# stresearch/xfr

Hardware: AMD Instinct MI355X
Metric: triplet-contrastive-EBP saliency maps/sec, ResNet-101 224x224 (higher is better)
Workload: dtype f32

## Files before the change

### xfr_amd/csrc/conv_gemm.hip

```cpp
#include <algorithm>
#include <atomic>
#include <mutex>
#include <unordered_map>
#include <vector>
#include "common.h"
#include <cstdio>
#include <cstdlib>

#include "conv_gemm_dev.h"
#include "conv_gemm_host.h"

std::atomic<long> g_conv_chain_launches[2];

namespace {

#ifndef XFR_MFM_WAVES
#define XFR_MFM_WAVES 6
#endif
#ifndef XFR_DUAL_WAVES
#define XFR_DUAL_WAVES 4
#endif
template <int TCO, int TM, int BK, int NST, int MODE, bool RELU, int CHAIN>
__global__ __launch_bounds__(NT, CHAIN == 0 ? 1 : (CHAIN == 1 ? 7 : (CHAIN == 4 ? XFR_DUAL_WAVES : XFR_MFM_WAVES))) void conv_gemm_kernel(const ConvParams p, const int n_co_tiles, const int n_m_tiles)
{
// ... 491 lines not shown
            if (kk + 2 < BK) {
#pragma unroll
                for (int i = 0; i < 2; ++i) { a_nxt[i] = As[(kk + 2 + lhi) * TCO + l31 + i * 32]; b_nxt[i] = Bs[(kk + 2 + lhi) * TM + l31 + i * 32]; }
            } else {
                wait_vmcnt<(NST - 2) * L>();
                const float* An = ring + st_next * STAGE;
#pragma unroll
                for (int i = 0; i < 2; ++i) { a_nxt[i] = An[lhi * TCO + l31 + i * 32]; b_nxt[i] = An[A_FLOATS + lhi * TM + l31 + i * 32]; }
            }
            if (RELU) { b_cur[0] = fmaxf(b_cur[0], 0.f); b_cur[1] = fmaxf(b_cur[1], 0.f); }
#pragma unroll
            for (int i = 0; i < 2; ++i)
#pragma unroll
                for (int j = 0; j < 2; ++j) acc[i][j] = __builtin_amdgcn_mfma_f32_32x32x2f32(a_cur[i], b_cur[j], acc[i][j], 0, 0, 0);
            if constexpr (DUAL) {
                const float ap0 = fmaxf(a_cur[0], 0.f), ap1 = fmaxf(a_cur[1], 0.f);
#pragma unroll
                for (int j = 0; j < 2; ++j) {
                    accp[0][j] = __builtin_amdgcn_mfma_f32_32x32x2f32(ap0, b_cur[j], accp[0][j], 0, 0, 0);
                    accp[1][j] = __builtin_amdgcn_mfma_f32_32x32x2f32(ap1, b_cur[j], accp[1][j], 0, 0, 0);
                }
            }
            if (kk + 2 < BK) issue(kt + NST - 1, st_fill, kk / 2);
            __builtin_amdgcn_sched_group_barrier(0x100, 2, 0);
            __builtin_amdgcn_sched_group_barrier(0x008, 1, 0);
            __builtin_amdgcn_sched_group_barrier(0x020, (L + NP - 1) / NP, 0);
            __builtin_amdgcn_sched_group_barrier(0x008, DUAL ? 7 : 3, 0);
#pragma unroll
            for (int i = 0; i < 2; ++i) { a_cur[i] = a_nxt[i]; b_cur[i] = b_nxt[i]; }
        }
        st = st_next;
        asm volatile("" ::: "memory");
    }
    wait_vmcnt<0>();
    stamp(p, wave, lane, 2);

    asm volatile("s_waitcnt lgkmcnt(0)" ::: "memory");
    v16f accq[1][1];
    if (wave == 0) ks_exchange<0, WAVE_LDS>(smem, acc, lane, accq[0][0]);
    else if (wave == 1) ks_exchange<1, WAVE_LDS>(smem, acc, lane, accq[0][0]);
    else if (wave == 2) ks_exchange<2, WAVE_LDS>(smem, acc, lane, accq[0][0]);
    else ks_exchange<3, WAVE_LDS>(smem, acc, lane, accq[0][0]);
    v16f accpq;
    if constexpr (DUAL) {
        __syncthreads();
        if (wave == 0) ks_exchange<0, WAVE_LDS>(smem, accp, lane, accpq);
        else if (wave == 1) ks_exchange<1, WAVE_LDS>(smem, accp, lane, accpq);
        else if (wave == 2) ks_exchange<2, WAVE_LDS>(smem, accp, lane, accpq);
        else ks_exchange<3, WAVE_LDS>(smem, accp, lane, accpq);
    }
    stamp(p, wave, lane, 3);
    block_epilogue<CHAIN, true>(p, accq, smem, tid, lane, wave, co0, m0, half, tail_t, part, nparts, osel, bsel, DUAL ? &accpq : nullptr);
    stamp(p, wave, lane, 4);
}


int num_cus()
{
    static const int n = [] {
        int dev = 0, cu = 0;
        if (hipGetDevice(&dev) != hipSuccess || hipDeviceGetAttribute(&cu, hipDeviceAttributeMultiprocessorCount, dev) != hipSuccess || cu <= 0)
            cu = 256;
        return cu;
    }();
    return n;
}

int pick_tail_split(const ConvParams& p, int tiles, int nk, size_t tile_bytes)
{
    constexpr int qmax = 7;
    if (!p.tail_ws || !p.tail_cnt || p.tail_force == 1) return 1;
    const int C = num_cus();
    const int q = tiles / C, r = tiles % C;
    if (r == 0 || r > XFR_TAIL_MAX_TILES) return 1;
    const long max_blocks = (long)(p.tail_ws_bytes / tile_bytes);
    if (p.tail_force >= 2) {
        const int S = std::min(p.tail_force, nk);
        return ((long)r * S <= max_blocks) ? S : 1;
    }
    if (q == 0 && p.K >= 8192 && p.tail_force == 0) {
        const long S = std::min<long>(std::min<long>(64, p.K / 256), std::min<long>(max_blocks / r, std::max<long>(8, C / r)));
        return (int)std::min<long>(S, nk);
    }
    if (q >= qmax || p.K < 1024) return 1;
    const double ramp = 192.0 / (double)p.K;
    const double whole = 1.0 + ramp;
    double best = whole;
    int bestS = 1;
    const int Smax = std::min(std::min(8, p.K / 256), nk);
    for (int S = 2; S <= Smax; ++S) {
        if ((long)r * S > max_blocks) break;
        const double per_cu = (double)(((long)r * S + C - 1) / C);
        const double cost = per_cu * (1.0 / S + ramp) + 0.01 * S;
        if (cost < best) { best = cost; bestS = S; }
    }
    if (whole - best < 0.04 * (q + 1) * whole) bestS = 1;
    return bestS;
}

void warn_interpreted(const ConvParams& q)
{
    static std::atomic<int> said{0};
    const int ohw = q.OH * q.OW;
    const bool vec_ok = (q.M & 3) == 0 && ((q.chain_B * ohw) & 3) == 0 && ((q.out_nb * ohw) & 3) == 0;
    if (q.chain_interpret || !vec_ok || getenv("XFR_QUIET") || said.exchange(1)) return;
    uint16_t codes[XFR_MAX_EW_STEPS];
    const int n = ew_chain_codes(q.chain, codes);
    fprintf(stderr, "xfr_amd: a GEMM launch (Cout %d, K %d, M %d) runs its %d-step fused chain through the INTERPRETED epilogue: no compiled signature [", q.CoutTot, q.K, q.M, q.chain.n);
    for (int i = 0; i < n; ++i) fprintf(stderr, "%s%04x", i ? " " : "", codes[i]);
    fprintf(stderr, "]%s.  Regenerate the table (python tools/gen_chain_sigs.py && make -C xfr_amd/csrc) if this network is a supported backbone; "
                    "xfr_chain_epilogue_stats counts such launches.  (said once; XFR_QUIET=1 silences it)\n",
            n < 0 ? " (the chain carries a trace / prior / capture: interpreted by design)" : (q.accumulate ? " for an accumulating launch" : ""));
}

int plan_chain(ConvParams& q)
{
    EwChain wide = q.chain;
    EwLoads wide_ld;
    ew_plan_loads(wide, q.out0, wide_ld, EW_FWD_SLOTS_WIDE);
    ew_plan_loads(q.chain, q.out0, q.chain_ld);
    const int ohw = q.OH * q.OW;
    const bool vec_ok = (q.M & 3) == 0 && ((q.chain_B * ohw) & 3) == 0 && ((q.out_nb * ohw) & 3) == 0;
    q.chain_sig = (q.accumulate || !vec_ok || q.chain_interpret) ? -1 : conv_gemm_chain_sig(wide);
    if (q.chain_sig >= 0) { q.chain = wide; q.chain_ld = wide_ld; }
    if (q.nhalves == 2 && q.chain_sig < 0) return 1;
    if ((q.dualacc != 0) != (q.chain_sig >= 0 && chain_sig_is_dual(q.chain_sig))) return 3;
    for (int i = 0; i < q.chain.n && q.chain_sig < 0; ++i)
        if (q.chain.s[i].type == EW_MAXPAIR || q.chain.s[i].type == EW_MAXHALF_OUT) return 2;
    return 0;
}

template <int TCO, int TM, int BK, int NST, int MODE>
bool launch_one(const ConvParams& p, hipStream_t s)
{
    const int n_co = ((p.CoutTot + TCO - 1) / TCO) * p.nhalves;
    const int n_m = (p.M + TM - 1) / TM;
    const size_t lds = std::max((size_t)NST * BK * (TCO + TM) * sizeof(float) + (MODE == MODE_GEN ? 512 * sizeof(int2) : 0), (size_t)4 * 32 * 36 * sizeof(float));
    ConvParams q = p;
    int grid = n_co * n_m;
    q.tail_q = 0;
    q.tail_s = 1;
    {
        const int S = pick_tail_split(p, n_co * n_m, (p.K + BK - 1) / BK, (size_t)TCO * TM * sizeof(float) * (p.dualacc ? 2 : 1));
        if (S > 1) {
            const int r = (n_co * n_m) % num_cus();
            q.tail_q = n_co * n_m - r;
            q.tail_s = S;
            grid = q.tail_q + r * S;
        }
    }
    if (p.dualacc && (q.chain.n == 0 || p.nhalves != 1 || p.relu_in)) return false;
    if constexpr ((TCO == 64 && TM == 64) || (TCO == 32 && TM == 128)) {
        if (q.chain.n > 0) {
            if (plan_chain(q)) return false;
            g_conv_chain_launches[q.chain_sig >= 0 ? 0 : 1]++;
            if (q.chain_sig < 0) warn_interpreted(q);
            if constexpr (TCO == 64 && MODE != MODE_TAP4 && MODE != MODE_GEN) {
                if (q.dualacc) {
                    hipLaunchKernelGGL((conv_gemm_kernel<TCO, TM, BK, NST, MODE, false, 4>), dim3(grid), dim3(NT), lds, s, q, n_co, n_m);
                    return true;
                }
            }
            if (q.dualacc) return false;
            if (q.chain_sig >= 0 && chain_sig_is_mfm(q.chain_sig))
                hipLaunchKernelGGL((conv_gemm_kernel<TCO, TM, BK, NST, MODE, false, 3>), dim3(grid), dim3(NT), lds, s, q, n_co, n_m);
            else if (q.chain_sig >= 0)
                hipLaunchKernelGGL((conv_gemm_kernel<TCO, TM, BK, NST, MODE, false, 1>), dim3(grid), dim3(NT), lds, s, q, n_co, n_m);
            else
                hipLaunchKernelGGL((conv_gemm_kernel<TCO, TM, BK, NST, MODE, false, 2>), dim3(grid), dim3(NT), lds, s, q, n_co, n_m);
            return true;
        }
    }
    if (p.relu_in)
        hipLaunchKernelGGL((conv_gemm_kernel<TCO, TM, BK, NST, MODE, true, 0>), dim3(grid), dim3(NT), lds, s, q, n_co, n_m);
    else
        hipLaunchKernelGGL((conv_gemm_kernel<TCO, TM, BK, NST, MODE, false, 0>), dim3(grid), dim3(NT), lds, s, q, n_co, n_m);
    return true;
}

template <int BK, int NST, int MODE>
bool launch_one_ks(const ConvParams& p, hipStream_t s)
{
    constexpr int TCO = 64, TM = 64;
    const int n_co = ((p.CoutTot + TCO - 1) / TCO) * p.nhalves;
    const int n_m = (p.M + TM - 1) / TM;
    constexpr int RING = NST * BK * (TCO + TM);
    const size_t lds = (size_t)4 * (RING > 2048 ? RING : 2048) * sizeof(float);
    ConvParams q = p;
    int grid = n_co * n_m;
    q.tail_q = 0;
    q.tail_s = 1;
    {
        const int S = pick_tail_split(p, n_co * n_m, (p.K + BK - 1) / BK, (size_t)TCO * TM * sizeof(float) * (p.dualacc ? 2 : 1));
        if (S > 1) {
            const int r = (n_co * n_m) % num_cus();
            q.tail_q = n_co * n_m - r;
            q.tail_s = S;
            grid = q.tail_q + r * S;
        }
    }
    if (p.dualacc && (q.chain.n == 0 || p.nhalves != 1 || p.relu_in)) return false;
    if (q.chain.n > 0) {
        if (plan_chain(q)) return false;
        g_conv_chain_launches[q.chain_sig >= 0 ? 0 : 1]++;
        if (q.chain_sig < 0) warn_interpreted(q);
        if (q.dualacc) {
            hipLaunchKernelGGL((conv_gemm_ks_kernel<BK, NST, MODE, false, 4>), dim3(grid), dim3(NT), lds, s, q, n_co, n_m);
            return true;
        }
        if (q.chain_sig >= 0 && chain_sig_is_mfm(q.chain_sig))
            hipLaunchKernelGGL((conv_gemm_ks_kernel<BK, NST, MODE, false, 3>), dim3(grid), dim3(NT), lds, s, q, n_co, n_m);
        else if (q.chain_sig >= 0)
            hipLaunchKernelGGL((conv_gemm_ks_kernel<BK, NST, MODE, false, 1>), dim3(grid), dim3(NT), lds, s, q, n_co, n_m);
        else
            hipLaunchKernelGGL((conv_gemm_ks_kernel<BK, NST, MODE, false, 2>), dim3(grid), dim3(NT), lds, s, q, n_co, n_m);
        return true;
    }
    if (p.relu_in)
        hipLaunchKernelGGL((conv_gemm_ks_kernel<BK, NST, MODE, true, 0>), dim3(grid), dim3(NT), lds, s, q, n_co, n_m);
    else
        hipLaunchKernelGGL((conv_gemm_ks_kernel<BK, NST, MODE, false, 0>), dim3(grid), dim3(NT), lds, s, q, n_co, n_m);
    return true;
}

template <int BK>
bool ks_ok(const ConvParams& p)
{
    if ((p.Cin % BK) != 0) return false;
    if (p.kh == 1 && p.kw == 1) return p.pad == 0 && p.stride <= 2;
    if (p.out_stride != 1) return false;
    return p.stride == 1 && p.tap_major == 1 && p.kh * p.kw <= 64;
}

template <int BK, int NST>
bool launch_cfg_ks(const ConvParams& p, hipStream_t s)
{
    const bool vec = (p.kh == 1 && p.kw == 1 && p.stride == 1 && p.pad == 0 && (p.M % 4) == 0 && p.OH == p.H && p.OW == p.W);
    if (vec) return launch_one_ks<BK, NST, MODE_VEC>(p, s);
    return launch_one_ks<BK, NST, MODE_TAP>(p, s);
}


template <int TCO, int TM, int BK, int NST>
bool launch_cfg(const ConvParams& p_in, hipStream_t s)
{
    ConvParams p = p_in;
    if (p.dualacc && p.kh == 1 && p.kw == 1 && p.tap_major == 0 && (p.Cin % 16) == 0) p.tap_major = 1;
    const bool vec = (p.kh == 1 && p.kw == 1 && p.stride == 1 && p.pad == 0 && (p.M % 4) == 0 && p.OH == p.H && p.OW == p.W);
    if (vec) return launch_one<TCO, TM, BK, NST, MODE_VEC>(p, s);
    if (p.tap_major == 2) return launch_one<64, 64, 16, 4, MODE_TAP4>(p, s);
    if (p.tap_major && (p.Cin % BK) == 0) return launch_one<TCO, TM, BK, NST, MODE_TAP>(p, s);
    if (p.tap_major) return launch_one<TCO, TM, 16, 4, MODE_TAP>(p, s);
    return launch_one<TCO, TM, 16, 4, MODE_GEN>(p, s);
}

}

int conv_gemm_num_cus() { return num_cus(); }
int conv_gemm_plan_chain(ConvParams& q) { return plan_chain(q); }
void conv_gemm_warn_interpreted(const ConvParams& q) { warn_interpreted(q); }

int conv_gemm_chain_sig(const EwChain& ch)
{
    uint16_t codes[XFR_MAX_EW_STEPS];
    const int n = ew_chain_codes(ch, codes);
    if (n <= 0) return -1;
    for (int sgi = 0; sgi < kNumChainSigs; ++sgi) {
        bool same = true;
        for (int i = 0; i < XFR_MAX_EW_STEPS && same; ++i) same = kChainSigs[sgi][i] == (i < n ? codes[i] : 0);
        if (same) return sgi;
    }
    return -1;
}
int conv_gemm_num_chain_sigs() { return kNumChainSigs; }

int conv_gemm_cannot_launch(const ConvParams& p)
{
    if (p.chain.n <= 0) return 0;
    ConvParams q = p;
    return plan_chain(q);
}
const char* conv_gemm_refusal(int why)
{
    switch (why) {
        case 0: return "the convolution launch was refused without a reason";
        case 1: return "a dual (W / relu(W)) convolution launch carries a fused chain without a compiled epilogue";
        case 3: return "lean probe-forward steps and the dual-accumulator launch (ConvParams::dualacc) only exist together, behind a compiled epilogue";
        case 2: return "a fused chain with a MaxFeatureMap step (pair maximum / fan-out VJP) has no compiled epilogue and the interpreter does not run those steps";
        default: return "unknown convolution launch refusal";
    }
}

void conv_gemm_chain_launch_counts(long* compiled, long* interpreted)
{
    if (compiled) *compiled = g_conv_chain_launches[0].load();
    if (interpreted) *interpreted = g_conv_chain_launches[1].load();
}

static int pick_cfg_impl(const ConvParams& p_in, bool allow_split);
int conv_gemm_pick_cfg(const ConvParams& p_in) { return pick_cfg_impl(p_in, true); }
static int pick_cfg_impl(const ConvParams& p_in, bool allow_split)
{
    ConvParams p = p_in;
    if (p.dualacc) { p.nhalves = 2; p.dualacc = 0; const int c = pick_cfg_impl(p, false); return c == 12 ? 4 : c; }
    if (allow_split && p.split_ok && conv_gemm_split_wanted(p)) return 9;
    {
        const int rem = p.CoutTot % 64;
#ifndef XFR_NO_ROW_TILE
        if (rem > 0 && rem <= 32 && p.tap_major != 2 && p.out_stride == 1 && p.CoutTot > 32 && p.M > 64) return 12;
#endif
    }
    if (ks_ok<8>(p)) {
        if (p.kh == 1 && (p.stride == 2 || p.out_stride == 2 || p.as_strided)) return 7;
        if ((p.kh > 1 && p.K >= 2048) || (p.kh == 1 && (p.K == 512 || p.K >= 2048))) return 7;
    }
    const long tiles = (long)((p.CoutTot + 63) / 64) * p.nhalves * ((p.M + 63) / 64);
    if (p.K >= 1024 && tiles <= 512 && (p.tap_major ? (p.Cin % 32 == 0) : true)) return 5;
    return 4;
}

static std::mutex g_tune_mu;
static thread_local int g_last_cfg = 0;
static std::atomic<int> g_tuning{0};
static unsigned long long* g_stamps = nullptr;
static int g_stamps_cap = 0;
static int g_stamp_regions = 0, g_stamp_seq = 0;
namespace {
struct LogRec { void* stream; int cout, nhalves, K, M, kh, chain, cfg; };
unsigned long long* g_log = nullptr;
int g_log_cap = 0;
std::vector<LogRec> g_log_recs;
bool g_log_on() { return g_log != nullptr; }
}
void conv_gemm_set_stamps(unsigned long long* dev_ptr, int capacity_workgroups)
{
    std::lock_guard<std::mutex> lk(g_tune_mu);
    g_stamps = dev_ptr;
    g_stamps_cap = dev_ptr ? (capacity_workgroups < 0 ? -capacity_workgroups : capacity_workgroups) : 0;
    g_stamp_regions = (dev_ptr && capacity_workgroups < 0) ? (-capacity_workgroups) / 256 : 0;
    g_stamp_seq = 0;
    g_tuning.store((g_stamps || g_log_on()) ? 1 : 0);
}

void conv_gemm_set_log(unsigned long long* log_dev, int capacity)
{
    std::lock_guard<std::mutex> lk(g_tune_mu);
    g_log = log_dev;
    g_log_cap = log_dev ? capacity : 0;
    g_log_recs.clear();
    g_tuning.store((g_stamps || g_log) ? 1 : 0);
}
int conv_gemm_dump_log(const char* path)
{
    std::lock_guard<std::mutex> lk(g_tune_mu);
    if (!g_log) return 0;
    const size_t n = g_log_recs.size();
    std::vector<unsigned long long> h(8 * n + 8);
    if (n && hipMemcpy(h.data(), g_log, 8 * n * sizeof(unsigned long long), hipMemcpyDeviceToHost) != hipSuccess) return -1;
    FILE* f = fopen(path, "w");
    if (!f) return -1;
    fprintf(f, "seq,stream,Cout,nhalves,K,M,kh,chain,cfg,start_10ns,end_10ns\n");
    for (size_t i = 0; i < n; ++i) {
        const LogRec& r = g_log_recs[i];
        fprintf(f, "%zu,%p,%d,%d,%d,%d,%d,%d,%d,%llu,%llu\n", i, r.stream, r.cout, r.nhalves, r.K, r.M, r.kh, r.chain, r.cfg, h[8 * i], *std::max_element(h.begin() + 8 * i + 1, h.begin() + 8 * i + 8));
    }
    fclose(f);
    return (int)n;
}

bool launch_conv_gemm(const ConvParams& p_in, hipStream_t s)
{
    ConvParams p = p_in;
    p.stamps = nullptr;
    p.stamps_cap = 0;
    p.stamp_regions = 0;
    p.stamp_seq = 0;
    p.span = nullptr;
    size_t log_idx = (size_t)-1;
    if (g_tuning.load(std::memory_order_relaxed)) {
        std::lock_guard<std::mutex> lk(g_tune_mu);
        p.stamps = g_stamps;
        p.stamps_cap = g_stamps_cap;
        p.stamp_regions = g_stamp_regions;
        p.stamp_seq = g_stamps ? g_stamp_seq++ : 0;
        if (g_log && (int)g_log_recs.size() < g_log_cap) {
            p.span = g_log + 8 * g_log_recs.size();
            log_idx = g_log_recs.size();
            g_log_recs.push_back(LogRec{(void*)s, p.CoutTot, p.dualacc ? 2 : p.nhalves, p.K, p.M, p.kh, p.chain.n, -1});
        }
    }
    int cfg = p.force_cfg > 0 ? p.force_cfg : conv_gemm_pick_cfg(p);
    {
        struct Remap { int v[32]; };
        static const Remap remap = [] {
            Remap r;
            for (int i = 0; i < 32; ++i) r.v[i] = i;
            if (const char* e = getenv("XFR_CFG_REMAP")) {
                int a = 0, b = 0, n = 0;
                while (sscanf(e, "%d:%d%n", &a, &b, &n) == 2) {
                    if (a >= 0 && a < 32 && b >= 0 && b < 32) r.v[a] = b;
                    e += n;
                    if (*e == ',') ++e;
                }
            }
            return r;
        }();
        if (p.force_cfg <= 0 && cfg >= 0 && cfg < 32) cfg = remap.v[cfg];
    }
    auto ran = [&](int eff, bool ok) {
        g_last_cfg = eff;
        if (log_idx != (size_t)-1) {
            std::lock_guard<std::mutex> lk(g_tune_mu);
            if (log_idx < g_log_recs.size()) g_log_recs[log_idx].cfg = eff;
        }
        return ok;
    };
    if (cfg == 9) {
        if (conv_gemm_launch_split(p, s)) return ran(9, true);
        cfg = pick_cfg_impl(p, false);
    }
    if (cfg == 6 && ks_ok<8>(p)) return ran(6, launch_cfg_ks<8, 3>(p, s));
    if (cfg == 7 && ks_ok<4>(p)) return ran(7, launch_cfg_ks<4, 4>(p, s));
    if (cfg == 5) return ran(5, launch_cfg<64, 64, 32, 3>(p, s));
    if (cfg == 12) return ran(12, launch_cfg<32, 128, 16, 3>(p, s));
    return ran(4, launch_cfg<64, 64, 16, 3>(p, s));
}

int conv_gemm_last_cfg() { return g_last_cfg; }
```

### xfr_amd/csrc/conv_gemm_split.hip

```cpp
#include <algorithm>
#include <atomic>
#include <mutex>
#include <unordered_map>
#include <cstdio>
#include <cstdlib>
#include <type_traits>
#include "conv_gemm_dev.h"
#include "conv_gemm_host.h"

namespace {

typedef __bf16 v8bf __attribute__((ext_vector_type(8)));
typedef unsigned v4u __attribute__((ext_vector_type(4)));
constexpr int SP_T = 128, SP_BK = 16;
constexpr int SP_A_BYTES = 3 * 2 * SP_T * 16, SP_B_BYTES = 3 * 2 * SP_T * 16;
constexpr size_t SP_LDS = 3 * (size_t)(SP_A_BYTES + SP_B_BYTES);

typedef float v2f_t __attribute__((ext_vector_type(2)));
typedef __bf16 v2bf_t __attribute__((ext_vector_type(2)));
__device__ __forceinline__ unsigned cvt_pk_bf16(float lo, float hi)
{
    const v2f_t t = {lo, hi};
    return __builtin_bit_cast(unsigned, __builtin_convertvector(t, v2bf_t));
}
__device__ __forceinline__ void split_pair(float a, float b, unsigned& p0, unsigned& p1, unsigned& p2)
{
    p0 = cvt_pk_bf16(a, b);
    const float ra = a - __uint_as_float(p0 << 16), rb = b - __uint_as_float(p0 & 0xffff0000u);
    p1 = cvt_pk_bf16(ra, rb);
    const float sa = ra - __uint_as_float(p1 << 16), sb = rb - __uint_as_float(p1 & 0xffff0000u);
    p2 = cvt_pk_bf16(sa, sb);
}

constexpr int SPP_MAX_HALO = 64, SPP_MAX_TAPS = 25;

__host__ __device__ inline int spp_halo(const ConvParams& p) { return p.pad * p.W + p.pad; }
__host__ __device__ inline int spp_patch_len(const ConvParams& p) { return SP_T + 2 * spp_halo(p); }
inline size_t spp_lds_bytes(const ConvParams& p) { return (size_t)3 * SP_A_BYTES + (size_t)2 * 6 * (spp_patch_len(p) + 1) * 16; }

constexpr int NT8 = 512;

template <int N>
__device__ __forceinline__ void sp8_wait_barrier()
{
    asm volatile("s_waitcnt vmcnt(%0) lgkmcnt(0)\n\ts_barrier" ::"n"(N) : "memory");
}

template <bool RELU, int CHAIN, bool PATCH>
__global__ __launch_bounds__(NT8, 2) void conv_gemm_split_kernel(const ConvParams p, const uint16_t* __restrict__ ws0, const uint16_t* __restrict__ ws1,
                                                                  const int n_co_tiles, const int n_m_tiles)
{
    extern __shared__ __attribute__((aligned(16))) float smem[];
    unsigned char* lds = reinterpret_cast<unsigned char*>(smem);
    constexpr int NST = 3, D = NST - 1, XBASE = NST * SP_A_BYTES;
    const int tid = threadIdx.x, lane = tid & 63, wave8 = __builtin_amdgcn_readfirstlane(tid >> 6);
    const int wr4 = wave8 >> 1, wc = wave8 & 1;
    const int l31 = lane & 31, lhi = lane >> 5;
    const bool two_dma = wave8 < 4;
    if (wave8 < 4) stamp(p, wave8, lane, 0, 4);

    const int lid = xcd_remap(blockIdx.x, n_co_tiles * n_m_tiles);
    const int tile_m = lid / n_co_tiles;
    const int tile_co_all = lid - tile_m * n_co_tiles;
    const int n_co_half = n_co_tiles / p.nhalves;
    const int half = tile_co_all / n_co_half;
    const int tile_co = tile_co_all - half * n_co_half;
    const int co0 = tile_co * SP_T, m0 = tile_m * SP_T;
    const uint16_t* __restrict__ wsel = half ? ws1 : ws0;
    const float* __restrict__ bsel = half ? p.bias_pos : p.bias;
    float* __restrict__ osel = half ? p.out1 : p.out0;
    const int T = p.kh * p.kw, ncb = p.Cin / SP_BK, nk = p.K / SP_BK;
    const int halo = spp_halo(p), PL = spp_patch_len(p);
    const int PS = PATCH ? (PL + 1) * 16 : SP_T * 16;
    const int XB = 6 * PS;
    const unsigned chan_bytes = (unsigned)p.in_nb * p.H * p.W * 4u;
    const __amdgpu_buffer_rsrc_t rW = __builtin_amdgcn_make_buffer_rsrc((void*)wsel, 0, n_co_half * nk * SP_A_BYTES, 0x00020000);
    const __amdgpu_buffer_rsrc_t rIn = __builtin_amdgcn_make_buffer_rsrc((void*)p.in, 0, (int)p.in_bytes, 0x00020000);
    const unsigned lds_base = (unsigned)(size_t)(__attribute__((address_space(3))) unsigned char*)(lds);

    unsigned t_voff = OOB, t_lds = 0;
    bool t_ok = false;
    int base_m = 0;
    unsigned long long tapmask = 0ull;
    const int sm = tid & 127, skq = wave8 >> 1;
    if constexpr (PATCH) {
        const int kh_ = tid >= PL ? 1 : 0, q = tid - kh_ * PL;
        const long g = (long)m0 - halo + q;
        t_ok = tid < 2 * PL;
        const bool in_row = t_ok && g >= 0 && g < (long)p.in_nb * p.H * p.W;
        t_voff = in_row ? (unsigned)g * 4u + (unsigned)(kh_ * 8) * chan_bytes : OOB;
        t_lds = lds_base + XBASE + kh_ * PS + q * 16;
    } else {
        const int m = m0 + sm;
        const bool m_ok = m < p.M;
        const int mm = m_ok ? m : 0;
        const int ohw = p.OH * p.OW;
        const int n = mm / ohw;
        const int r = mm - n * ohw;
        const int oh = r / p.OW;
        const int ow = r - oh * p.OW;
        const int ih0 = oh * p.stride - p.pad, iw0 = ow * p.stride - p.pad;
        base_m = n * p.H * p.W + ih0 * p.W + iw0;
        if (m_ok) {
            unsigned long long vw = 0ull;
            for (int dw = 0; dw < p.kw; ++dw)
                if ((unsigned)(iw0 + dw) < (unsigned)p.W) vw |= 1ull << dw;
            for (int dh = 0; dh < p.kh; ++dh)
                if ((unsigned)(ih0 + dh) < (unsigned)p.H) tapmask |= vw << (dh * p.kw);
        }
        t_lds = lds_base + XBASE + ((skq >> 1) * SP_T + sm) * 16 + (skq & 1) * 8;
    }
    int c_pos[2] = {0, 0};
    unsigned c_mask[2] = {0u, 0u};
    if constexpr (PATCH) {
#pragma unroll
        for (int j = 0; j < 2; ++j) {
            const int c = wc * 64 + j * 32 + l31, m = m0 + c;
            c_pos[j] = c + halo;
            unsigned mk = 0u;
            if (m < p.M) {
                const int ohw = p.OH * p.OW;
                const int r = m % ohw;
                const int oh = r / p.OW, ow = r - oh * p.OW;
                for (int dh = 0; dh < p.kh; ++dh)
                    for (int dw = 0; dw < p.kw; ++dw)
                        if ((unsigned)(oh + dh - p.pad) < (unsigned)p.H && (unsigned)(ow + dw - p.pad) < (unsigned)p.W) mk |= 1u << (dh * p.kw + dw);
            }
            c_mask[j] = mk;
        }
    }
    const unsigned char* a_lane = lds + (lhi * SP_T + wr4 * 32 + l31) * 16;
    const unsigned char* b_plane = lds + XBASE + lhi * PS;

    v16f acc[2], pipe[2];
#pragma unroll
    for (int j = 0; j < 2; ++j)
#pragma unroll
        for (int r = 0; r < 16; ++r) { acc[j][r] = 0.f; pipe[j][r] = 0.f; }

    auto dma = [&](int kt, int stage, int ch) {
        __builtin_amdgcn_raw_ptr_buffer_load_lds(rW, (lptr_t)(lds + stage * SP_A_BYTES + ch * 1024), 16, (ch * 1024 + lane * 16) | (kt < nk ? 0u : OOB),
                                                 (tile_co * nk + kt) * SP_A_BYTES, 0, 0);
    };
    auto load_w = [&](int kt, int stage) {
        dma(kt, stage, wave8);
        if (two_dma) dma(kt, stage, 8 + wave8);
    };
    auto fold = [&](bool negated) {
        if (negated) { acc[0] -= pipe[0]; acc[1] -= pipe[1]; }
        else { acc[0] += pipe[0]; acc[1] += pipe[1]; }
    };
    auto mfmas = [&](const v8bf (&af)[3], const v8bf (&bf)[3][2], auto FIRST) {
        constexpr int TA[6] = {2, 1, 0, 1, 0, 0}, TB[6] = {0, 1, 2, 0, 1, 0};
        v16f zero;
#pragma unroll
        for (int r = 0; r < 16; ++r) zero[r] = 0.f;
#pragma unroll
        for (int t = 0; t < 6; ++t)
#pragma unroll
            for (int j = 0; j < 2; ++j)
                pipe[j] = __builtin_amdgcn_mfma_f32_32x32x16_bf16(af[TA[t]], bf[TB[t]][j], (t == 0 && decltype(FIRST)::value) ? zero : pipe[j], 0, 0, 0);
    };
    std::integral_constant<int, 0> S0; std::integral_constant<int, 1> S1; std::integral_constant<int, 2> S2;
    std::integral_constant<bool, true> first; std::integral_constant<bool, false> later;

    if constexpr (PATCH) {
        float xp[8];
        auto load_patch = [&](int cb) {
            const unsigned so = (unsigned)(cb * SP_BK) * chan_bytes;
#pragma unroll
            for (int i = 0; i < 8; ++i) xp[i] = __uint_as_float(__builtin_amdgcn_raw_buffer_load_b32(rIn, t_voff, so + (unsigned)i * chan_bytes, 0));
        };
        auto store_patch = [&](int buf, unsigned flip) {
            v4u q0, q1, q2;
#pragma unroll
            for (int i = 0; i < 4; ++i) {
                const float a = RELU ? fmaxf(xp[2 * i], 0.f) : xp[2 * i], b = RELU ? fmaxf(xp[2 * i + 1], 0.f) : xp[2 * i + 1];
                unsigned h0, h1, h2;
                split_pair(a, b, h0, h1, h2);
                q0[i] = h0 ^ flip; q1[i] = h1 ^ flip; q2[i] = h2 ^ flip;
            }
            if (t_ok) {
                const unsigned at = t_lds + buf * XB;
                asm volatile("ds_write_b128 %0, %1" :: "v"(at), "v"(q0));
                asm volatile("ds_write_b128 %0, %1" :: "v"(at + 2 * PS), "v"(q1));
                asm volatile("ds_write_b128 %0, %1" :: "v"(at + 4 * PS), "v"(q2));
            }
        };
        int tap = 0, cb = 0, buf = 0, shift = -halo, tdw = 0;
        bool xl_prev = false, xl_now = false;
        const bool mfma_first = wave8 < 4;
        auto load_part = [&](int kt, v8bf (&af)[3], v8bf (&bf)[3][2]) {
            const int st1 = (kt + 1) % 3, st3 = kt % 3;
            const bool more = cb + 1 < ncb;
            xl_now = false;
            if (more && tap == 2) store_patch(buf ^ 1, ((cb + 1) & 1) ? 0x80008000u : 0u);
            load_w(kt + 3, kt < 0 ? 2 : st3);
            if (more && tap == 0) { load_patch(cb + 1); xl_now = true; }
            const unsigned char* As = a_lane + (kt < 0 ? 0 : st1) * SP_A_BYTES;
#pragma unroll
            for (int pc = 0; pc < 3; ++pc) af[pc] = *(const v8bf*)(As + pc * 2 * SP_T * 16);
#pragma unroll
            for (int j = 0; j < 2; ++j) {
                const int pos = ((c_mask[j] >> tap) & 1u) ? c_pos[j] + shift : PL;
                const unsigned char* Bs = b_plane + buf * XB + pos * 16;
#pragma unroll
                for (int pc = 0; pc < 3; ++pc) bf[pc][j] = *(const v8bf*)(Bs + pc * 2 * PS);
            }
            tap += 1; tdw += 1; shift += 1;
            if (tdw == p.kw) { tdw = 0; shift += p.W - p.kw; }
            if (tap == T) { tap = 0; shift = -halo; cb += 1; buf ^= 1; }
        };
        auto end_step = [&]() {
            if (xl_now || xl_prev) { if (two_dma) sp8_wait_barrier<10>(); else sp8_wait_barrier<9>(); }
            else { if (two_dma) sp8_wait_barrier<2>(); else sp8_wait_barrier<1>(); }
            xl_prev = xl_now;
        };
        auto step = [&](int kt, v8bf (&caf)[3], v8bf (&cbf)[3][2], v8bf (&naf)[3], v8bf (&nbf)[3][2], auto FIRST) {
            if (mfma_first) mfmas(caf, cbf, FIRST);
            __builtin_amdgcn_sched_barrier(0);
            load_part(kt, naf, nbf);
            __builtin_amdgcn_sched_barrier(0);
            if (!mfma_first) mfmas(caf, cbf, FIRST);
            end_step();
        };
        if (tid < 12) {
            const v4u z = {0u, 0u, 0u, 0u};
            asm volatile("ds_write_b128 %0, %1" :: "v"(lds_base + XBASE + (tid / 6) * XB + (tid % 6) * PS + PL * 16), "v"(z));
        }
        load_w(0, 0);
        load_w(1, 1);
        load_patch(0);
        asm volatile("s_waitcnt vmcnt(0)" ::: "memory");
        store_patch(0, 0u);
        sp8_wait_barrier<0>();
        v8bf f0a[3], f0b[3][2], f1a[3], f1b[3][2];
        load_part(-1, f0a, f0b);
        end_step();
        if (wave8 < 4) stamp(p, wave8, lane, 1);
        int pass_in_blk = 0;
        bool neg = false;
        const int passes_per_blk = T / 3;
        auto pass_done = [&]() {
            fold(neg);
            if (++pass_in_blk == passes_per_blk) { pass_in_blk = 0; neg = !neg; }
        };
        for (int kt = 0; kt < nk; kt += 6) {
            step(kt, f0a, f0b, f1a, f1b, first);
            step(kt + 1, f1a, f1b, f0a, f0b, later);
            step(kt + 2, f0a, f0b, f1a, f1b, later);
            pass_done();
            step(kt + 3, f1a, f1b, f0a, f0b, first);
            step(kt + 4, f0a, f0b, f1a, f1b, later);
            step(kt + 5, f1a, f1b, f0a, f0b, later);
            pass_done();
        }
    } else {
        int ld_tap = 0, ld_ci0 = 0;
        unsigned ld_voff = (tapmask & 1ull) ? (unsigned)base_m * 4u : OOB;
        auto load_x = [&](int kt, float (&v)[4]) {
            const unsigned voff = ld_voff | (kt < nk ? 0u : OOB);
            const unsigned so = (unsigned)(ld_ci0 + skq * 4) * chan_bytes;
#pragma unroll
            for (int i = 0; i < 4; ++i) v[i] = __uint_as_float(__builtin_amdgcn_raw_buffer_load_b32(rIn, voff, so + (unsigned)i * chan_bytes, 0));
            ld_ci0 += SP_BK;
            if (ld_ci0 >= p.Cin) {
                ld_ci0 = 0;
                ld_tap += 1;
                const int dh = ld_tap / p.kw, dw = ld_tap - dh * p.kw;
                ld_voff = (ld_tap < p.kh * p.kw && ((tapmask >> ld_tap) & 1ull)) ? (unsigned)(base_m + dh * p.W + dw) * 4u : OOB;
            }
        };
        auto store_x = [&](const float (&v)[4], int stage, unsigned flip) {
            typedef unsigned v2u __attribute__((ext_vector_type(2)));
            v2u q0, q1, q2;
#pragma unroll
            for (int i = 0; i < 2; ++i) {
                const float a = RELU ? fmaxf(v[2 * i], 0.f) : v[2 * i], b = RELU ? fmaxf(v[2 * i + 1], 0.f) : v[2 * i + 1];
                unsigned h0, h1, h2;
                split_pair(a, b, h0, h1, h2);
                q0[i] = h0 ^ flip; q1[i] = h1 ^ flip; q2[i] = h2 ^ flip;
            }
            const unsigned at = t_lds + stage * XB;
            asm volatile("ds_write_b64 %0, %1" :: "v"(at), "v"(q0));
            asm volatile("ds_write_b64 %0, %1" :: "v"(at + 2 * PS), "v"(q1));
            asm volatile("ds_write_b64 %0, %1" :: "v"(at + 4 * PS), "v"(q2));
        };
        int wst = 0;
        auto step = [&](int kt, auto ST, float (&xcur)[4], float (&xnew)[4], unsigned flip, auto FIRST) {
            constexpr int st = decltype(ST)::value, st1 = (st + 1) % 3;
            const int stD = wst + D >= NST ? wst + D - NST : wst + D;
            load_w(kt + D, stD);
            load_x(kt + 3, xnew);
            const unsigned char* As = a_lane + wst * SP_A_BYTES;
            const unsigned char* Bs = b_plane + st * XB + (wc * 64 + l31) * 16;
            v8bf af[3], bf[3][2];
#pragma unroll
            for (int pc = 0; pc < 3; ++pc) {
                af[pc] = *(const v8bf*)(As + pc * 2 * SP_T * 16);
#pragma unroll
                for (int j = 0; j < 2; ++j) bf[pc][j] = *(const v8bf*)(Bs + pc * 2 * PS + j * 32 * 16);
            }
            mfmas(af, bf, FIRST);
            store_x(xcur, st1, flip);
            if (two_dma) sp8_wait_barrier<8 + 2 * (D - 1)>(); else sp8_wait_barrier<8 + (D - 1)>();
            wst = wst + 1 == NST ? 0 : wst + 1;
        };
        float x0[4], x1[4], x2[4];
        load_w(0, 0);
        load_x(0, x0);
        asm volatile("s_waitcnt vmcnt(0)" ::: "memory");
        store_x(x0, 0, 0u);
#pragma unroll
        for (int d = 1; d < D; ++d) load_w(d, d);
        load_x(1, x0);
        load_x(2, x1);
        if (two_dma) sp8_wait_barrier<8 + 2 * (D - 1)>(); else sp8_wait_barrier<8 + (D - 1)>();
        if (wave8 < 4) stamp(p, wave8, lane, 1);
        unsigned flip = 0u;
        for (int kt = 0; kt < nk; kt += 3) {
            const bool negated = flip != 0u;
            step(kt, S0, x0, x2, flip, first);
            step(kt + 1, S1, x1, x0, flip, later);
            flip ^= 0x80008000u;
            step(kt + 2, S2, x2, x1, flip, later);
            fold(negated);
        }
    }
    wait_vmcnt<0>();
    asm volatile("s_waitcnt lgkmcnt(0)" ::: "memory");
    if (wave8 < 4) { stamp(p, wave8, lane, 2); stamp(p, wave8, lane, 3); }

#pragma unroll 1
    for (int c = 0; c < 2; ++c) {
        v16f t[1][1];
        t[0][0] = acc[0];
        const int wq = (wr4 & 1) * 2 + c;
        block_epilogue<CHAIN, true>(p, t, smem + (wave8 - wq) * (32 * 36), tid & 255, lane, wq, co0 + (wr4 >> 1) * 64, m0 + wc * 64, half, -1, 0, 1, osel, bsel, nullptr);
        acc[0] = acc[1];
    }
    if (wave8 < 4) stamp(p, wave8, lane, 4);
}

__global__ void split_pack_kernel(const float* __restrict__ w, uint16_t* __restrict__ planes, int K, int cout, int ldw, int taps)
{
    const long idx = (long)blockIdx.x * blockDim.x + threadIdx.x;
    if (idx >= (long)K * cout) return;
    const int k = (int)(idx / cout), co = (int)(idx - (long)k * cout);
    unsigned h[3];
    split_pair(w[(long)k * ldw + co], 0.f, h[0], h[1], h[2]);
    const int cin = K / taps, tap = k / cin, ci = k - tap * cin;
    const int rt = co / SP_T, r = co - rt * SP_T, kt = (ci / SP_BK) * taps + tap, kk = ci % SP_BK, nk = K / SP_BK;
#pragma unroll
    for (int q = 0; q < 3; ++q)
        planes[((((long)(rt * nk + kt) * 3 + q) * 2 + kk / 8) * SP_T + r) * 8 + kk % 8] = (uint16_t)(h[q] & 0xffffu);
}

struct SplitPack { uint16_t* planes; int K, cout, ldw, taps; };
static std::mutex g_split_mu;
static std::unordered_map<const float*, SplitPack> g_split;

bool split_can_run(const ConvParams& p)
{
    if (p.dualacc || p.out_stride != 1 || p.as_strided || p.co_pair > 0 || p.stride != 1) return false;
    if ((p.Cin % SP_BK) != 0 || (p.K % SP_BK) != 0 || (p.CoutTot % SP_T) != 0) return false;
    if (p.kh == 1 && p.kw == 1) return p.pad == 0;
    return p.tap_major == 1 && p.kh * p.kw <= 64;
}
struct SplitPolicy { int min_k1, min_k3, min_tiles; };
const SplitPolicy& split_policy()
{
    static const SplitPolicy pol = [] {
        SplitPolicy q{256, 1152, 128};
        if (const char* e = getenv("XFR_SPLIT_MIN_K1")) q.min_k1 = atoi(e);
        if (const char* e = getenv("XFR_SPLIT_MIN_K3")) q.min_k3 = atoi(e);
        if (const char* e = getenv("XFR_SPLIT_MIN_TILES")) q.min_tiles = atoi(e);
        return q;
    }();
    return pol;
}
bool split_layer_ok(const ConvParams& p)
{
    if (!split_can_run(p)) return false;
    if (p.OH * p.OW < 196) return false;
    return p.K >= (p.kh == 1 && p.kw == 1 ? split_policy().min_k1 : split_policy().min_k3);
}
bool split_grid_ok(const ConvParams& p)
{
    const long tiles = (long)(p.CoutTot / SP_T) * p.nhalves * ((p.M + SP_T - 1) / SP_T);
    return tiles >= split_policy().min_tiles;
}

static std::atomic<long> g_split_launches{0};

bool split_patch_ok(const ConvParams& p)
{
    const int T = p.kh * p.kw;
    if (T < 5 || T > SPP_MAX_TAPS || (T % 3) != 0 || p.stride != 1 || p.tap_major != 1) return false;
    if (p.OH != p.H || p.OW != p.W || 2 * p.pad != p.kh - 1 || 2 * p.pad != p.kw - 1) return false;
    static const bool off = getenv("XFR_SPLIT_NO_PATCH") != nullptr;
    return spp_halo(p) <= SPP_MAX_HALO && !off;
}

const uint16_t* split_planes(const float* w, int K, int cout, int ldw, int taps, hipStream_t s)
{
    std::lock_guard<std::mutex> lk(g_split_mu);
    auto it = g_split.find(w);
    if (it != g_split.end())
        return (it->second.K == K && it->second.cout == cout && it->second.ldw == ldw && it->second.taps == taps) ? it->second.planes : nullptr;
    SplitPack sp{nullptr, K, cout, ldw, taps};
    if (hipMalloc(&sp.planes, (size_t)K * cout * 3 * sizeof(uint16_t)) != hipSuccess) {
        (void)hipGetLastError();
        sp.planes = nullptr;
        g_split[w] = sp;
        return nullptr;
    }
    const long n = (long)K * cout;
    hipLaunchKernelGGL(split_pack_kernel, dim3((unsigned)((n + 255) / 256)), dim3(256), 0, s, w, sp.planes, K, cout, ldw, taps);
    if (hipStreamSynchronize(s) != hipSuccess) { (void)hipFree(sp.planes); return nullptr; }
    g_split[w] = sp;
    return sp.planes;
}

template <bool RELU, int CHAIN>
void launch_split_inst(const ConvParams& q, const uint16_t* w0, const uint16_t* w1, int n_co, int n_m, hipStream_t s, bool patch)
{
    static std::atomic<unsigned long long> done{0ull};
    int dev = 0;
    (void)hipGetDevice(&dev);
    const unsigned long long bit = 1ull << (dev & 63);
    constexpr int PATCH_LDS_MAX = 3 * SP_A_BYTES + 2 * 6 * (SP_T + 2 * SPP_MAX_HALO + 1) * 16;
    if (!(done.load(std::memory_order_relaxed) & bit)) {
        (void)hipFuncSetAttribute((const void*)conv_gemm_split_kernel<RELU, CHAIN, false>, hipFuncAttributeMaxDynamicSharedMemorySize, (int)SP_LDS);
        (void)hipFuncSetAttribute((const void*)conv_gemm_split_kernel<RELU, CHAIN, true>, hipFuncAttributeMaxDynamicSharedMemorySize, PATCH_LDS_MAX);
        done.fetch_or(bit);
    }
    const dim3 grid(n_co * n_m);
    if (patch) hipLaunchKernelGGL((conv_gemm_split_kernel<RELU, CHAIN, true>), grid, dim3(NT8), spp_lds_bytes(q), s, q, w0, w1, n_co, n_m);
    else hipLaunchKernelGGL((conv_gemm_split_kernel<RELU, CHAIN, false>), grid, dim3(NT8), SP_LDS, s, q, w0, w1, n_co, n_m);
}

bool launch_split(const ConvParams& p, hipStream_t s)
{
    if (p.force_cfg == 9 ? !split_can_run(p) : !conv_gemm_split_wanted(p)) return false;
    if (p.chain.n > 0 && p.relu_in) return false;
    ConvParams q = p;
    q.tail_q = 0;
    q.tail_s = 1;
    int family = p.relu_in ? -1 : 0;
    if (q.chain.n > 0) {
        if (conv_gemm_plan_chain(q)) return false;
        if (q.chain_sig >= 0 && chain_sig_is_dual(q.chain_sig)) return false;
        family = q.chain_sig < 0 ? 2 : (chain_sig_is_mfm(q.chain_sig) ? 3 : 1);
    }
    const bool patch = split_patch_ok(p);
    const int taps = patch ? p.kh * p.kw : 1;
    const uint16_t* w0 = split_planes(p.w, p.K, p.CoutTot, p.ldw, taps, s);
    const uint16_t* w1 = p.nhalves == 2 ? split_planes(p.w_pos, p.K, p.CoutTot, p.ldw, taps, s) : nullptr;
    if (!w0 || (p.nhalves == 2 && !w1)) return false;
    g_split_launches++;
    if (q.chain.n > 0) {
        g_conv_chain_launches[q.chain_sig >= 0 ? 0 : 1]++;
        if (q.chain_sig < 0) conv_gemm_warn_interpreted(q);
    }
    const int n_co = (p.CoutTot / SP_T) * p.nhalves;
    const int n_m = (p.M + SP_T - 1) / SP_T;
    switch (family) {
        case -1: launch_split_inst<true, 0>(q, w0, w1, n_co, n_m, s, patch); break;
        case 0: launch_split_inst<false, 0>(q, w0, w1, n_co, n_m, s, patch); break;
        case 1: launch_split_inst<false, 1>(q, w0, w1, n_co, n_m, s, patch); break;
        case 2: launch_split_inst<false, 2>(q, w0, w1, n_co, n_m, s, patch); break;
        default: launch_split_inst<false, 3>(q, w0, w1, n_co, n_m, s, patch); break;
    }
    return true;
}

}

void conv_gemm_forget_split(const void* lo, size_t bytes)
{
    std::lock_guard<std::mutex> lk(g_split_mu);
    const char* a = static_cast<const char*>(lo);
    for (auto it = g_split.begin(); it != g_split.end();) {
        const char* w = reinterpret_cast<const char*>(it->first);
        if (w >= a && w < a + bytes) {
            if (it->second.planes) (void)hipFree(it->second.planes);
            it = g_split.erase(it);
        } else ++it;
    }
}
int conv_gemm_split_covers(const ConvParams& p) { return split_layer_ok(p) ? 1 : 0; }
bool conv_gemm_presplit(const ConvParams& p, const float* w, hipStream_t s) { return split_planes(w, p.K, p.CoutTot, p.ldw, split_patch_ok(p) ? p.kh * p.kw : 1, s) != nullptr; }
bool conv_gemm_split_wanted(const ConvParams& p) { return split_layer_ok(p) && (p.split_ok == 2 || split_grid_ok(p)); }
bool conv_gemm_launch_split(const ConvParams& p, hipStream_t s) { return launch_split(p, s); }
long conv_gemm_split_launches() { return g_split_launches.load(); }
```

Measured before the change: 1567.

## Run dual-accumulator (W / relu(W)) convolutions through the bf16x3 split MFMA kernel

Adds a DUAL mode (CHAIN==4) to the split-precision convolution kernel. It keeps a second set of accumulators computed from relu-masked copies of the weight fragments, so one launch yields both the W and relu(W) products for the dual epilogue. The config picker now routes dualacc layers to the split path, where before they fell back to the older kernels. The change also widens the zero padding row in the patch LDS so masked taps spread over 16 zero slots, and it makes all waves issue MFMAs first in dual mode. In exchange, dual mode doubles the MFMA work and the accumulator registers, which may hurt occupancy.

```diff
diff --git a/xfr_amd/csrc/conv_gemm.hip b/xfr_amd/csrc/conv_gemm.hip
--- a/xfr_amd/csrc/conv_gemm.hip
+++ b/xfr_amd/csrc/conv_gemm.hip
@@ -817,6 +817,7 @@
 static int pick_cfg_impl(const ConvParams& p_in, bool allow_split)
 {
     ConvParams p = p_in;
+    if (p.dualacc && allow_split && p.split_ok && conv_gemm_split_wanted(p)) return 9;
     if (p.dualacc) { p.nhalves = 2; p.dualacc = 0; const int c = pick_cfg_impl(p, false); return c == 12 ? 4 : c; }
     if (allow_split && p.split_ok && conv_gemm_split_wanted(p)) return 9;
     {
diff --git a/xfr_amd/csrc/conv_gemm_split.hip b/xfr_amd/csrc/conv_gemm_split.hip
--- a/xfr_amd/csrc/conv_gemm_split.hip
+++ b/xfr_amd/csrc/conv_gemm_split.hip
@@ -32,13 +32,15 @@
     p2 = cvt_pk_bf16(sa, sb);
 }
 
+constexpr int NT8 = 512;
+
 constexpr int SPP_MAX_HALO = 64, SPP_MAX_TAPS = 25;
 
 __host__ __device__ inline int spp_halo(const ConvParams& p) { return p.pad * p.W + p.pad; }
 __host__ __device__ inline int spp_patch_len(const ConvParams& p) { return SP_T + 2 * spp_halo(p); }
-inline size_t spp_lds_bytes(const ConvParams& p) { return (size_t)3 * SP_A_BYTES + (size_t)2 * 6 * (spp_patch_len(p) + 1) * 16; }
-
-constexpr int NT8 = 512;
+constexpr int SPP_ZERO = 16;
+inline size_t spp_lds_bytes(const ConvParams& p) { return (size_t)3 * SP_A_BYTES + (size_t)2 * 6 * (spp_patch_len(p) + SPP_ZERO) * 16; }
+constexpr size_t SP_EPI_LDS = (size_t)(NT8 / 64) * 32 * 36 * sizeof(float);
 
 template <int N>
 __device__ __forceinline__ void sp8_wait_barrier()
@@ -53,6 +55,7 @@
     extern __shared__ __attribute__((aligned(16))) float smem[];
     unsigned char* lds = reinterpret_cast<unsigned char*>(smem);
     constexpr int NST = 3, D = NST - 1, XBASE = NST * SP_A_BYTES;
+    constexpr bool DUAL = CHAIN == 4;
     const int tid = threadIdx.x, lane = tid & 63, wave8 = __builtin_amdgcn_readfirstlane(tid >> 6);
     const int wr4 = wave8 >> 1, wc = wave8 & 1;
     const int l31 = lane & 31, lhi = lane >> 5;
@@ -71,7 +74,7 @@
     float* __restrict__ osel = half ? p.out1 : p.out0;
     const int T = p.kh * p.kw, ncb = p.Cin / SP_BK, nk = p.K / SP_BK;
     const int halo = spp_halo(p), PL = spp_patch_len(p);
-    const int PS = PATCH ? (PL + 1) * 16 : SP_T * 16;
+    const int PS = PATCH ? (PL + SPP_ZERO) * 16 : SP_T * 16;
     const int XB = 6 * PS;
     const unsigned chan_bytes = (unsigned)p.in_nb * p.H * p.W * 4u;
     const __amdgpu_buffer_rsrc_t rW = __builtin_amdgcn_make_buffer_rsrc((void*)wsel, 0, n_co_half * nk * SP_A_BYTES, 0x00020000);
@@ -132,11 +135,11 @@
     const unsigned char* a_lane = lds + (lhi * SP_T + wr4 * 32 + l31) * 16;
     const unsigned char* b_plane = lds + XBASE + lhi * PS;
 
-    v16f acc[2], pipe[2];
+    v16f acc[2], pipe[2], accp[2], pipep[2];
 #pragma unroll
     for (int j = 0; j < 2; ++j)
 #pragma unroll
-        for (int r = 0; r < 16; ++r) { acc[j][r] = 0.f; pipe[j][r] = 0.f; }
+        for (int r = 0; r < 16; ++r) { acc[j][r] = 0.f; pipe[j][r] = 0.f; accp[j][r] = 0.f; pipep[j][r] = 0.f; }
 
     auto dma = [&](int kt, int stage, int ch) {
         __builtin_amdgcn_raw_ptr_buffer_load_lds(rW, (lptr_t)(lds + stage * SP_A_BYTES + ch * 1024), 16, (ch * 1024 + lane * 16) | (kt < nk ? 0u : OOB),
@@ -149,17 +152,36 @@
     auto fold = [&](bool negated) {
         if (negated) { acc[0] -= pipe[0]; acc[1] -= pipe[1]; }
         else { acc[0] += pipe[0]; acc[1] += pipe[1]; }
+        if constexpr (DUAL) {
+            if (negated) { accp[0] -= pipep[0]; accp[1] -= pipep[1]; }
+            else { accp[0] += pipep[0]; accp[1] += pipep[1]; }
+        }
     };
     auto mfmas = [&](const v8bf (&af)[3], const v8bf (&bf)[3][2], auto FIRST) {
         constexpr int TA[6] = {2, 1, 0, 1, 0, 0}, TB[6] = {0, 1, 2, 0, 1, 0};
         v16f zero;
 #pragma unroll
         for (int r = 0; r < 16; ++r) zero[r] = 0.f;
-#pragma unroll
-        for (int t = 0; t < 6; ++t)
-#pragma unroll
-            for (int j = 0; j < 2; ++j)
-                pipe[j] = __builtin_amdgcn_mfma_f32_32x32x16_bf16(af[TA[t]], bf[TB[t]][j], (t == 0 && decltype(FIRST)::value) ? zero : pipe[j], 0, 0, 0);
+        if constexpr (DUAL) {
+            typedef short v8s __attribute__((ext_vector_type(8)));
+            const v8s neg = __builtin_bit_cast(v8s, af[0]) >> 15;
+            v8bf ap[3];
+#pragma unroll
+            for (int pc = 0; pc < 3; ++pc) ap[pc] = __builtin_bit_cast(v8bf, __builtin_bit_cast(v8s, af[pc]) & ~neg);
+#pragma unroll
+            for (int t = 0; t < 6; ++t)
+#pragma unroll
+                for (int j = 0; j < 2; ++j) {
+                    pipe[j] = __builtin_amdgcn_mfma_f32_32x32x16_bf16(af[TA[t]], bf[TB[t]][j], (t == 0 && decltype(FIRST)::value) ? zero : pipe[j], 0, 0, 0);
+                    pipep[j] = __builtin_amdgcn_mfma_f32_32x32x16_bf16(ap[TA[t]], bf[TB[t]][j], (t == 0 && decltype(FIRST)::value) ? zero : pipep[j], 0, 0, 0);
+                }
+        } else {
+#pragma unroll
+            for (int t = 0; t < 6; ++t)
+#pragma unroll
+                for (int j = 0; j < 2; ++j)
+                    pipe[j] = __builtin_amdgcn_mfma_f32_32x32x16_bf16(af[TA[t]], bf[TB[t]][j], (t == 0 && decltype(FIRST)::value) ? zero : pipe[j], 0, 0, 0);
+        }
     };
     std::integral_constant<int, 0> S0; std::integral_constant<int, 1> S1; std::integral_constant<int, 2> S2;
     std::integral_constant<bool, true> first; std::integral_constant<bool, false> later;
@@ -189,7 +211,7 @@
         };
         int tap = 0, cb = 0, buf = 0, shift = -halo, tdw = 0;
         bool xl_prev = false, xl_now = false;
-        const bool mfma_first = wave8 < 4;
+        const bool mfma_first = DUAL || wave8 < 4;
         auto load_part = [&](int kt, v8bf (&af)[3], v8bf (&bf)[3][2]) {
             const int st1 = (kt + 1) % 3, st3 = kt % 3;
             const bool more = cb + 1 < ncb;
@@ -202,7 +224,8 @@
             for (int pc = 0; pc < 3; ++pc) af[pc] = *(const v8bf*)(As + pc * 2 * SP_T * 16);
 #pragma unroll
             for (int j = 0; j < 2; ++j) {
-                const int pos = ((c_mask[j] >> tap) & 1u) ? c_pos[j] + shift : PL;
+                const int at = c_pos[j] + shift;
+                const int pos = ((c_mask[j] >> tap) & 1u) ? at : PL + ((at - PL) & (SPP_ZERO - 1));
                 const unsigned char* Bs = b_plane + buf * XB + pos * 16;
 #pragma unroll
                 for (int pc = 0; pc < 3; ++pc) bf[pc][j] = *(const v8bf*)(Bs + pc * 2 * PS);
@@ -224,9 +247,10 @@
             if (!mfma_first) mfmas(caf, cbf, FIRST);
             end_step();
         };
-        if (tid < 12) {
+        if (tid < 12 * SPP_ZERO) {
             const v4u z = {0u, 0u, 0u, 0u};
-            asm volatile("ds_write_b128 %0, %1" :: "v"(lds_base + XBASE + (tid / 6) * XB + (tid % 6) * PS + PL * 16), "v"(z));
+            const int pl = tid / SPP_ZERO;
+            asm volatile("ds_write_b128 %0, %1" :: "v"(lds_base + XBASE + (pl / 6) * XB + (pl % 6) * PS + (PL + tid % SPP_ZERO) * 16), "v"(z));
         }
         load_w(0, 0);
         load_w(1, 1);
@@ -234,7 +258,9 @@
         asm volatile("s_waitcnt vmcnt(0)" ::: "memory");
         store_patch(0, 0u);
         sp8_wait_barrier<0>();
-        v8bf f0a[3], f0b[3][2], f1a[3], f1b[3][2];
+        v8bf f0a[3], f0b[3][2], g1a[3], g1b[3][2];
+        v8bf (&f1a)[3] = DUAL ? f0a : g1a;
+        v8bf (&f1b)[3][2] = DUAL ? f0b : g1b;
         load_part(-1, f0a, f0b);
         end_step();
         if (wave8 < 4) stamp(p, wave8, lane, 1);
@@ -333,11 +359,14 @@
 
 #pragma unroll 1
     for (int c = 0; c < 2; ++c) {
-        v16f t[1][1];
+        v16f t[1][1], tp;
         t[0][0] = acc[0];
+        tp = accp[0];
         const int wq = (wr4 & 1) * 2 + c;
-        block_epilogue<CHAIN, true>(p, t, smem + (wave8 - wq) * (32 * 36), tid & 255, lane, wq, co0 + (wr4 >> 1) * 64, m0 + wc * 64, half, -1, 0, 1, osel, bsel, nullptr);
+        block_epilogue<CHAIN, true>(p, t, smem + (wave8 - wq) * (32 * 36), tid & 255, lane, wq, co0 + (wr4 >> 1) * 64, m0 + wc * 64, half, -1, 0, 1, osel, bsel,
+                                    DUAL ? &tp : nullptr);
         acc[0] = acc[1];
+        accp[0] = accp[1];
     }
     if (wave8 < 4) stamp(p, wave8, lane, 4);
 }
@@ -362,7 +391,8 @@
 
 bool split_can_run(const ConvParams& p)
 {
-    if (p.dualacc || p.out_stride != 1 || p.as_strided || p.co_pair > 0 || p.stride != 1) return false;
+    if (p.out_stride != 1 || p.as_strided || p.co_pair > 0 || p.stride != 1) return false;
+    if (p.dualacc && (p.nhalves != 1 || p.relu_in || p.chain.n == 0)) return false;
     if ((p.Cin % SP_BK) != 0 || (p.K % SP_BK) != 0 || (p.CoutTot % SP_T) != 0) return false;
     if (p.kh == 1 && p.kw == 1) return p.pad == 0;
     return p.tap_major == 1 && p.kh * p.kw <= 64;
@@ -429,7 +459,8 @@
     int dev = 0;
     (void)hipGetDevice(&dev);
     const unsigned long long bit = 1ull << (dev & 63);
-    constexpr int PATCH_LDS_MAX = 3 * SP_A_BYTES + 2 * 6 * (SP_T + 2 * SPP_MAX_HALO + 1) * 16;
+    constexpr int PATCH_LDS_MAX = 3 * SP_A_BYTES + 2 * 6 * (SP_T + 2 * SPP_MAX_HALO + SPP_ZERO) * 16;
+    static_assert(SP_LDS >= SP_EPI_LDS && 3 * SP_A_BYTES >= SP_EPI_LDS, "the epilogue tiles fit the LDS of both modes");
     if (!(done.load(std::memory_order_relaxed) & bit)) {
         (void)hipFuncSetAttribute((const void*)conv_gemm_split_kernel<RELU, CHAIN, false>, hipFuncAttributeMaxDynamicSharedMemorySize, (int)SP_LDS);
         (void)hipFuncSetAttribute((const void*)conv_gemm_split_kernel<RELU, CHAIN, true>, hipFuncAttributeMaxDynamicSharedMemorySize, PATCH_LDS_MAX);
@@ -450,9 +481,11 @@
     int family = p.relu_in ? -1 : 0;
     if (q.chain.n > 0) {
         if (conv_gemm_plan_chain(q)) return false;
-        if (q.chain_sig >= 0 && chain_sig_is_dual(q.chain_sig)) return false;
-        family = q.chain_sig < 0 ? 2 : (chain_sig_is_mfm(q.chain_sig) ? 3 : 1);
-    }
+        if (q.dualacc) {
+            if (q.chain_sig < 0 || !chain_sig_is_dual(q.chain_sig) || q.nhalves != 1) return false;
+            family = 4;
+        } else family = q.chain_sig < 0 ? 2 : (chain_sig_is_mfm(q.chain_sig) ? 3 : 1);
+    } else if (q.dualacc) return false;
     const bool patch = split_patch_ok(p);
     const int taps = patch ? p.kh * p.kw : 1;
     const uint16_t* w0 = split_planes(p.w, p.K, p.CoutTot, p.ldw, taps, s);
@@ -470,6 +503,7 @@
         case 0: launch_split_inst<false, 0>(q, w0, w1, n_co, n_m, s, patch); break;
         case 1: launch_split_inst<false, 1>(q, w0, w1, n_co, n_m, s, patch); break;
         case 2: launch_split_inst<false, 2>(q, w0, w1, n_co, n_m, s, patch); break;
+        case 4: launch_split_inst<false, 4>(q, w0, w1, n_co, n_m, s, patch); break;
         default: launch_split_inst<false, 3>(q, w0, w1, n_co, n_m, s, patch); break;
     }
     return true;
```

New measurement: 1589, median of 6. 1.01x the previous value.
